# Tw6249/dgppo_fov

Hardware: AMD Instinct MI355X
Metric: env-steps/sec + PPO-updates/sec, LidarSpread n=8 ×4096 envs, 1/2/4/8 GPU (higher is better)
Workload: dtype f32; 1 GPU; LidarSpread n=8 obs=3 rays=32 top_k=8, 4096 envs/GPU, 1 step = reset + T=128 fused env steps into the (B,T+1) rollout buffer; env=LidarSpread, num_agents=8, n_obs=3, n_env_per_gpu=4096, T=128, hip_graph=True, stream_lanes=1, persistent_rollout=True, parallelism=dp1 (env-sharded, no collective)

## Files before the change

### dgppo_fov_amd/_lib.py

```python
from __future__ import annotations

import ctypes
import os
import pathlib

PKG_DIR = pathlib.Path(__file__).resolve().parent
LIB_PATH = pathlib.Path(os.environ.get("DGPPO_HIP_LIB", PKG_DIR / "lib" / "libdgppo_hip.so"))

DGPPO_EINVAL = -22
DGPPO_ENGINE_LIDAR, DGPPO_ENGINE_BICYCLE, DGPPO_ENGINE_MPE, DGPPO_ENGINE_OMNI = 0, 1, 2, 3
DGPPO_ENGINE_VMAS_WHEEL, DGPPO_ENGINE_VMAS_TRANSPORT = 4, 5
DGPPO_VMAS_FIELDS = 8
DGPPO_GOAL_SPREAD, DGPPO_GOAL_TARGET = 0, 1
(DGPPO_VARIANT_NONE, DGPPO_VARIANT_LINE, DGPPO_VARIANT_FORMATION, DGPPO_VARIANT_CORRIDOR,
 DGPPO_VARIANT_CONNECT) = 0, 1, 2, 3, 4
DGPPO_OBST_FIELDS = 16

c_f32p = ctypes.c_void_p


class NativeLibraryError(RuntimeError):
    pass


# ... 163 lines not shown

class GemmPlan(ctypes.Structure):
    _fields_ = [(n, ctypes.c_int32) for n in ("path", "form", "ntw", "ncg", "nch", "vec", "extra", "epi", "mt", "nt",
                                               "unroll", "flat", "pipe", "chunks", "split_k", "grid")] + \
               [("units", ctypes.c_int64), ("lds_bytes", ctypes.c_int64)]


class GruSeqArgs(ctypes.Structure):
    _fields_ = [
        ("Q", ctypes.c_int32), ("L", ctypes.c_int32), ("n_agents", ctypes.c_int32), ("H", ctypes.c_int32),
        ("gi", c_f32p), ("Wh", c_f32p), ("bhn", c_f32p), ("h0", c_f32p), ("hs", c_f32p), ("hT", c_f32p),
        ("dhs", c_f32p), ("dgi", c_f32p), ("dgh", c_f32p), ("dh0", c_f32p), ("dbhn_part", c_f32p),
    ]


class GtLayer(ctypes.Structure):
    _fields_ = [("Wq", c_f32p), ("bq", c_f32p), ("Wkt", c_f32p), ("bk", c_f32p), ("Wcat", c_f32p), ("Wu", c_f32p),
                ("bu", c_f32p), ("D", ctypes.c_int32), ("F", ctypes.c_int32), ("Wex", c_f32p)]


class PolicyStepArgs(ctypes.Structure):
    _fields_ = [
        ("G", ctypes.c_int32), ("N", ctypes.c_int32), ("E", ctypes.c_int32), ("n_agents", ctypes.c_int32),
        ("C", ctypes.c_int32), ("D0", ctypes.c_int32), ("A", ctypes.c_int32), ("n_layers", ctypes.c_int32),
        ("H", ctypes.c_int32), ("mode", ctypes.c_int32), ("ED", ctypes.c_int32), ("pad_", ctypes.c_int32),
        ("cand", c_f32p),
        ("nodes", c_f32p), ("nodes_gstride", ctypes.c_int64),
        ("edges", c_f32p), ("edges_gstride", ctypes.c_int64),
        ("receivers", c_f32p), ("senders", c_f32p), ("idx_gstride", ctypes.c_int64),
        ("layer", GtLayer * 2),
# ... 135 lines not shown
    "dgppo_policy_step_supported": (ctypes.c_int, [_V]),
    "dgppo_policy_work_floats": (ctypes.c_int64, []),
    "dgppo_policy_prepare": (ctypes.c_int, [_V, _V]),
    "dgppo_policy_step": (ctypes.c_int, [_V, _V]),
    "dgppo_gnn_sender_table": (ctypes.c_int, [_I32, _I32, _I32, _I32, _V, _V, _V, _V, _V]),
    "dgppo_cost_shaped_loss": (ctypes.c_int, [_V, _V, ctypes.c_float, _V, _I32, _I32, _I32, _I32, _V]),
    "dgppo_informarl_advantages": (ctypes.c_int, [_V, _V, _V, _I32, _I32, _I32, _V]),
    "dgppo_gnn_edge_wsum": (ctypes.c_int, [_I32, _I32, _I32, _I32, _I32, _I32, _V, _V, _V, _V, _V, _V]),
    "dgppo_gnn_edge_da": (ctypes.c_int, [_I32, _I32, _I32, _I32, _I32, _I32, _V, _V, _V, _V, _V, _V]),
    "dgppo_gru_seq_fwd": (ctypes.c_int, [_V, _V]),
    "dgppo_gru_seq_bwd": (ctypes.c_int, [_V, _V]),
    "dgppo_agent_mean_fwd": (ctypes.c_int, [_V, _V, _I64, _I32, _I32, _I64, _V]),
    "dgppo_agent_mean_bwd": (ctypes.c_int, [_V, _V, _I64, _I32, _I32, _I64, _V]),
    "dgppo_agent_mean_bwd_masked": (ctypes.c_int, [_V, _V, _V, _I64, _I32, _I32, _I64, _V]),
    "dgppo_gru_set_form": (ctypes.c_int, [_I32]),
    "dgppo_gnn_set_graph_otf": (ctypes.c_int, [_I32]),
    "dgppo_tanh_normal": (ctypes.c_int, [ctypes.POINTER(TanhNormalArgs), ctypes.c_void_p]),
    "dgppo_loss_workspace_floats": (ctypes.c_int64, []),
    "dgppo_ppo_loss": (ctypes.c_int, [_V, _V, _V, _V, _I64, _F32, _F32, _V, _V, _V, _V, _V]),
    "dgppo_l2_loss": (ctypes.c_int, [_V, _V, _I64, _V, _V, _V, _V]),
    "dgppo_gae": (ctypes.c_int, [ctypes.POINTER(GaeArgs), ctypes.c_void_p]),
    "dgppo_dgppo_advantages": (ctypes.c_int, [ctypes.POINTER(AdvArgs), ctypes.c_void_p]),
    "dgppo_grad_norm": (ctypes.c_int, [_V, _I64, _V, _V, _V]),
    "dgppo_adam": (ctypes.c_int, [_V, _V, _V, _V, _I64, _V, _F32, ctypes.c_double, ctypes.c_double, _F32, _F32, _V]),
    "dgppo_adam_multi_workspace_floats": (ctypes.c_int64, []),
    "dgppo_adam_multi": (ctypes.c_int, [_V, _V]),
    "dgppo_normal": (ctypes.c_int, [_V, _I64, _V, ctypes.c_uint64, ctypes.c_uint64, _V]),
    "dgppo_clip_min0": (ctypes.c_int, [_V, _V, _I64, _V]),
    "dgppo_lagr_advantages": (ctypes.c_int, [_V, _V, _V, _V, _V, _V, _V, _I32, _I32, _I32, _I32, _V]),
    "dgppo_lagr_update": (ctypes.c_int, [_V, _V, _V, _V, _V, _V, _I64, _I32, _I32, _F32, _F32, _V]),
# ... 62 lines not shown
```

### dgppo_fov_amd/algo/module/nets.py

```python
from __future__ import annotations

import ctypes
import math
import os

import numpy as np
import torch

from ... import _lib
from ...nn import kernels as K
from ...nn.layers import FUSE_LN, GNN, Dense, GraphBatch, MLPHead, ParamSpace, RNNStack

VH_TAIL = os.environ.get("DGPPO_VH_TAIL", "0") == "1"
STD_DEV_INIT_INV = math.log(math.exp(0.5) - 1.0)
STD_DEV_MIN = 1e-5


class _Net:
    modules: list

    def init_host(self, seed: int):
        rng = np.random.default_rng(seed)
        for m in self.modules:
            m.init_host(rng)

    @property
# ... 103 lines not shown
        feat, h2, _ = self.gru.fwd(y, h, h_out=h_out)
        _, mu, sr = self._outputs(feat)
        action = action_out if action_out is not None else torch.empty((rows, self.A), device=h.device)
        log_pi = log_pi_out if log_pi_out is not None else torch.empty(rows, device=h.device)
        a = _lib.TanhNormalArgs()
        a.rows, a.A, a.mode, a.n_agents = rows, self.A, mode, self.n
        a.mean, a.std_raw = K._p(mu), K._p(sr)
        a.std_shift, a.std_min = STD_DEV_INIT_INV, STD_DEV_MIN
        a.noise = K._p(noise)
        a.action_out, a.log_pi = K._p(action), K._p(log_pi)
        K.tanh_normal(a, h.device)
        return action, log_pi, h2

    def eval_seq_fwd(self, g: GraphBatch, S: int, L: int, actions: torch.Tensor, entropy_eps: torch.Tensor):
        n, dev = self.n, actions.device
        y, tc = self._trunk(g)
        H2, gcs = self.gru.seq_fwd(y, S * n, L, n)
        s, mu, sr = self._outputs(H2)
        rows = S * L * n
        log_pi = torch.empty(rows, device=dev)
        ent = torch.empty(rows, device=dev)
        a = _lib.TanhNormalArgs()
        a.rows, a.A, a.mode, a.n_agents = rows, self.A, 2, n
        a.mean, a.std_raw, a.action = K._p(mu), K._p(sr), K._p(actions)
        a.std_shift, a.std_min = STD_DEV_INIT_INV, STD_DEV_MIN
        a.log_pi, a.entropy, a.entropy_eps = K._p(log_pi), K._p(ent), K._p(entropy_eps)
        K.tanh_normal(a, dev)
        cache = (g, S, L, tc, gcs, H2, s, mu, sr, actions, entropy_eps)
        return log_pi, ent, cache

    def eval_seq_bwd(self, cache, dlog_pi, dentropy):
        g, S, L, tc, gcs, H2, s, mu, sr, actions, entropy_eps = cache
# ... 3 lines not shown
        dsr = torch.empty_like(sr)
        a = _lib.TanhNormalArgs()
        a.rows, a.A, a.mode, a.n_agents = rows, self.A, 2, n
        a.mean, a.std_raw, a.action = K._p(mu), K._p(sr), K._p(actions)
        a.std_shift, a.std_min = STD_DEV_INIT_INV, STD_DEV_MIN
        a.entropy_eps = K._p(entropy_eps)
        a.dlog_pi, a.dentropy, a.dmean, a.dstd_raw = K._p(dlog_pi), K._p(dentropy), K._p(dmu), K._p(dsr)
        K.tanh_normal(a, dev)
        ds = self.mean.bwd(s, dmu, rows)
        self.std.bwd(s, dsr, rows, dx_out=ds, accumulate=True)
        dH2 = self.scale_hid.bwd(H2, ds, rows)
        self._bptt(dH2.view(S, L, n, 64), gcs, S, L, tc, g)

    def _bptt(self, dHs, gcs, S, L, tc, g):
        gc, hc = tc
        ln = self.head.ln1_bwd_args(hc) if self.gru.simple else None
        dY, _ = self.gru.seq_bwd(gcs, dHs.reshape(S * L * self.n, 64), ln=ln)
        fused = ln is not None
        dz = self.head.bwd(hc, dY, dy_is_dh1=fused, mask_input=fused)
        self.gnn.bwd(gc, dz, g, top_masked=fused)


class VlNet(_Net):
    def __init__(self, node_dim: int, n_agents: int, device, seed: int = 1, gnn_layers: int = 2, edge_dim: int = 4,
                 rnn: str = "gru", rnn_layers: int = 1):
        self.n = n_agents
        ps = self.ps = ParamSpace()
        self.gnn = GNN(ps, "gnn", node_dim, gnn_layers, edge_dim=edge_dim)
        self.head = MLPHead(ps, "head")
        self.gru = RNNStack(ps, "gru", rnn, rnn_layers)
        self.out = Dense(ps, "out", 64, 1)
        self.modules = [self.gnn, self.head, self.gru, self.out]
        ps.build(device)
        self.init_host(seed)
# ... 13 lines not shown
        z, _ = self.gnn.fwd(g, keep=False)
        K.agent_mean_fwd(z, zm, g.G, self.n, 64, self.n * 64)
        return zm

    def seq_fwd(self, g: GraphBatch, S: int, L: int, h0=None, keep_cache=True, zm=None):
        dev = self.ps.flat.device
        G = S * L
        if zm is not None:
            assert not keep_cache, "seq_fwd from precomputed agent means is forward-only"
            z = gc = None
        else:
            n = self.n
            z, gc = self.gnn.fwd(g, keep=keep_cache)
            zm = torch.empty((G, 64), device=dev)
            K.agent_mean_fwd(z, zm, G, n, 64, n * 64)
        y, hc = self.head.fwd(zm)
        hT = torch.empty((S, self.gru.W), device=dev)
        Hs, gcs = self.gru.seq_fwd(y, S, L, 1, h0=h0, hT_out=hT)
        v = self.out.fwd(Hs, G)
        cache = (g, S, L, gc, z, hc, gcs, Hs) if keep_cache else None
        return v.view(S, L), hT, cache

    def seq_bwd(self, cache, dv):
        g, S, L, gc, z, hc, gcs, Hs = cache
        n, dev = self.n, dv.device
        G = S * L
        dH = self.out.bwd(Hs, dv.reshape(G, 1).contiguous(), G)
        ln = self.head.ln1_bwd_args(hc) if self.gru.simple else None
        dY, _ = self.gru.seq_bwd(gcs, dH, ln=ln)
        dzm = self.head.bwd(hc, dY, dy_is_dh1=ln is not None)
        dz = torch.empty_like(z)
        K.agent_mean_bwd(dzm, dz, G, n, 64, n * 64, mask=z if FUSE_LN else None)
        self.gnn.bwd(gc, dz, g, top_masked=FUSE_LN)


class VhNet(_Net):
    def __init__(self, node_dim: int, n_agents: int, n_cost: int, device, seed: int = 2, gnn_layers: int = 1,
                 edge_dim: int = 4, rnn: str = "gru", rnn_layers: int = 1):
        self.n, self.n_cost = n_agents, n_cost
        ps = self.ps = ParamSpace()
        self.gnn = GNN(ps, "gnn", node_dim, gnn_layers, edge_dim=edge_dim)
        self.head = MLPHead(ps, "head")
        self.gru = RNNStack(ps, "gru", rnn, rnn_layers)
        self.out = Dense(ps, "out", 64, n_cost)
        self.modules = [self.gnn, self.head, self.gru, self.out]
# ... 10 lines not shown

    def fwd(self, g: GraphBatch, h: torch.Tensor, keep_cache=True):
        rows = g.G * self.n
        self.last_tail = False
        if VH_TAIL and not keep_cache and self.gru.simple and len(self.gnn.layers) == 1 and h.shape[1] == 64:
            out = torch.empty((rows, self.n_cost), device=h.device)
            hd, cell = self.head, self.gru.cells[0]
            v = self.ps.view
            tail_w = [hd.d0.W(), hd.d0.b(), v(hd.ln0.name + ".scale"), v(hd.ln0.name + ".bias"), hd.d1.W(), hd.d1.b(),
                      v(hd.ln1.name + ".scale"), v(hd.ln1.name + ".bias"), cell.v("Wi"), cell.v("bi"), cell.v("Wh"),
                      cell.v("bhn"), self.out.W(), self.out.b()]
            if self.gnn.fwd_epilogue(g, tail=(tail_w, h if h.is_contiguous() else h.contiguous(), out)) is not None:
                self.last_tail = True
                return out, None
        z, gc = self.gnn.fwd(g, keep=keep_cache)
        y, hc = self.head.fwd(z)
        h2, _, rc = self.gru.fwd(y, h)
        out = self.out.fwd(h2, rows)
        return out, ((g, gc, hc, rc, h2) if keep_cache else None)

    def bwd(self, cache, dout):
        g, gc, hc, rc, h2 = cache
        rows = g.G * self.n
        dh2 = self.out.bwd(h2, dout, rows)
        ln = self.head.ln1_bwd_args(hc) if self.gru.simple else None
        dy, _ = self.gru.seq_bwd(rc, dh2, ln=ln)
        fused = ln is not None
        dz = self.head.bwd(hc, dy, dy_is_dh1=fused, mask_input=fused)
        self.gnn.bwd(gc, dz, g, top_masked=fused)


class VhGlobalNet(_Net):

    def __init__(self, node_dim: int, n_agents: int, n_cost: int, device, seed: int = 2, gnn_layers: int = 1,
                 edge_dim: int = 4, rnn: str = "gru", rnn_layers: int = 1):
        self.n, self.n_cost = n_agents, n_cost
        ps = self.ps = ParamSpace()
        self.gnn = GNN(ps, "gnn", node_dim, gnn_layers, edge_dim=edge_dim)
        self.head = MLPHead(ps, "head", d_in=128)
        self.gru = RNNStack(ps, "gru", rnn, rnn_layers)
        self.out = Dense(ps, "out", 64, n_cost)
        self.modules = [self.gnn, self.head, self.gru, self.out]
        ps.build(device)
# ... 54 lines not shown
```

### dgppo_fov_amd/csrc/gemm.hip

```cpp
#include <hip/hip_runtime.h>
#include <stdint.h>
#include <stdlib.h>

#include "../../include/dgppo_hip.h"
#include "lanes.h"
#include "lds_attr.h"

namespace dgppo {

typedef float f32x16 __attribute__((ext_vector_type(16)));

constexpr int kBM = 64, kBN = 64, kBK = 32, kPitch = kBM + 1;

__device__ float4 g_zero_row[4];
__device__ float g_sink[64];

struct GemmTileArgs {
  int M, N, K, k_begin, k_end;
  bool ta, tb;
  const float* A;
  int64_t lda;
  const float* B;
  int64_t ldb;
  int a_grp, b_grp;
// ... 148 lines not shown
struct EpiAcc {
  float ds[NTW], db[NTW];
};

__device__ __forceinline__ float swz16(float v) {
  return __builtin_bit_cast(float, __builtin_amdgcn_ds_swizzle(__builtin_bit_cast(int, v), 0x401F));
}
__device__ __forceinline__ float red32(float v) {
  v = lanes::sum16(v);
  return v + swz16(v);
}
__device__ __forceinline__ void ln_stats(float v0, float v1, float& mean, float& rstd) {
#pragma clang fp contract(off)
  const float s1 = red32(v0 + v1);
  const float s2 = red32(v0 * v0 + v1 * v1);
  mean = s1 / 64.0f;
  float var = s2 / 64.0f - mean * mean;
  var = var > 0.0f ? var : 0.0f;
  rstd = 1.0f / sqrtf(var + 1e-6f);
}
__device__ __forceinline__ float ln_pre(float v, float mean, float rstd, float sc, float bi) {
#pragma clang fp contract(off)
  return ((v - mean) * rstd) * sc + bi;
}

template <int NTW, int EXTRA, int EPI>
__device__ __forceinline__ void epi_load(const dgppo_gemm_args& p, const float* C, const float* Dd, int m0, int col0,
                                         int i, int h, float (&bv)[NTW], float (&xv)[NTW][16], EpiX<NTW, EPI>& ex) {
#pragma clang fp contract(off)
  if (EPI == dgppo::kEpiLnBwd) {
    const int row = m0 + (i & 3) + 8 * ((i & 15) >> 2) + 4 * h;
    const bool ok = row < p.M;
    ex.mo = *(ok ? p.ln_mean + row : (const float*)g_zero_row);
    ex.ro = *(ok ? p.ln_rstd + row : (const float*)g_zero_row);
  }
#pragma unroll
  for (int t = 0; t < NTW; ++t) {
    const int col = col0 + 32 * t + i;
// ... 1179 lines not shown
```

### dgppo_fov_amd/nn/kernels.py

```python
from __future__ import annotations

import ctypes
import math
import weakref

import torch

from .. import _lib, ops

_WS = {}
_GRAPHS = weakref.WeakSet()
_WS_KEPT = []


def hold_for_graph(g):
    _GRAPHS.add(g)
    return g


def workspace(nfloats: int, device, slot: str = "default") -> torch.Tensor:
    key = (str(device), slot, _lib.stream_handle(device))
    t = _WS.get(key)
    if t is None or t.numel() < nfloats:
        old = t.numel() if t is not None else 0
# ... 212 lines not shown
    a = _lib.GruSeqArgs()
    a.Q, a.L, a.n_agents, a.H = int(Q), int(L), int(n), 64
    a.gi, a.Wh, a.bhn, a.h0, a.hs, a.hT = _p(gi), _p(Wh), _p(bhn), _p(h0), _p(hs), _p(hT)
    a.dhs, a.dgi, a.dgh, a.dh0, a.dbhn_part = _p(dhs), _p(dgi), _p(dgh), _p(dh0), _p(dbhn_part)
    lib = _lib.load()
    if fwd:
        _chk(lib.dgppo_gru_seq_fwd(ctypes.byref(a), _stream(hs)), "dgppo_gru_seq_fwd")
    else:
        _chk(lib.dgppo_gru_seq_bwd(ctypes.byref(a), _stream(hs)), "dgppo_gru_seq_bwd")


def gru_seq_blocks(Q):
    return int(_lib.load().dgppo_gru_seq_blocks(int(Q)))


def agent_mean_fwd(x, y, G, n, F, x_gstride):
    _chk(_lib.load().dgppo_agent_mean_fwd(_p(x), _p(y), int(G), int(n), int(F), int(x_gstride), _stream(y)),
         "dgppo_agent_mean_fwd")


def agent_mean_bwd(dy, dx, G, n, F, dx_gstride, mask=None):
    _chk(_lib.load().dgppo_agent_mean_bwd_masked(_p(dy), _p(mask), _p(dx), int(G), int(n), int(F), int(dx_gstride),
                                                 _stream(dx)), "dgppo_agent_mean_bwd_masked")


def sender_table(G, n, C, E, cand, receivers, senders, out):
    _chk(_lib.load().dgppo_gnn_sender_table(int(G), int(n), int(C), int(E), _p(cand), _p(receivers), _p(senders),
                                            _p(out), _stream(out)), "dgppo_gnn_sender_table")


# ... 99 lines not shown
```

### dgppo_fov_amd/nn/layers.py

```python
from __future__ import annotations

import math
import os
from typing import Dict, List, Optional, Tuple

import numpy as np
import torch

from .. import ops
from . import kernels as K

FUSE_LN = os.environ.get("DGPPO_FUSE_LN", "1") == "1"
FUSED_LAYER = os.environ.get("DGPPO_FUSED_LAYER", "1") == "1"


class ParamSpace:

    def __init__(self):
        self.entries: List[Tuple[str, Tuple[int, ...], str]] = []
        self.offsets: Dict[str, int] = {}
        self.size = 0
        self.flat = None
        self.grad = None

    def add(self, name: str, shape, init: str) -> str:
        shape = tuple(int(s) for s in shape)
        assert name not in self.offsets, name
        self.offsets[name] = self.size
# ... 222 lines not shown
        H = self.H
        wi, bi, wh, bhn = (self.v(k).cpu().numpy() for k in ("Wi", "bi", "Wh", "bhn"))
        return {"ir": {"kernel": wi[:, :H], "bias": bi[:H]}, "iz": {"kernel": wi[:, H:2 * H], "bias": bi[H:2 * H]},
                "in": {"kernel": wi[:, 2 * H:], "bias": bi[2 * H:]}, "hr": {"kernel": wh[:, :H]},
                "hz": {"kernel": wh[:, H:2 * H]}, "hn": {"kernel": wh[:, 2 * H:], "bias": bhn}}

    def load_flax(self, d):
        wi = np.concatenate([d["ir"]["kernel"], d["iz"]["kernel"], d["in"]["kernel"]], 1).astype(np.float32)
        bi = np.concatenate([d["ir"]["bias"], d["iz"]["bias"], d["in"]["bias"]]).astype(np.float32)
        wh = np.concatenate([d["hr"]["kernel"], d["hz"]["kernel"], d["hn"]["kernel"]], 1).astype(np.float32)
        self.v("Wi").copy_(torch.from_numpy(wi))
        self.v("bi").copy_(torch.from_numpy(bi))
        self.v("Wh").copy_(torch.from_numpy(wh))
        self.v("bhn").copy_(torch.as_tensor(np.asarray(d["hn"]["bias"], np.float32)))

    def seq_fwd(self, x, Q, L, n, h0=None, hs_out=None, hT_out=None):
        rows, H = Q * L, self.H
        gi = torch.empty((rows, 3 * H), device=x.device)
        K.gemm(x, self.v("Wi"), gi, rows, 3 * H, self.d_in, bias=self.v("bi"))
        hs = hs_out if hs_out is not None else torch.empty((rows, H), device=x.device)
        K.gru_seq(True, Q, L, n, gi, self.v("Wh"), self.v("bhn"), h0, hs, hT=hT_out)
        return hs, (x, gi, hs, h0, Q, L, n)

    def seq_bwd(self, cache, dhs, need_dx=True, need_dh0=False, ln=None):
        x, gi, hs, h0, Q, L, n = cache
        rows, H, dev = Q * L, self.H, dhs.device
        dgi = torch.empty((rows, 3 * H), device=dev)
        dgh = torch.empty((rows, 3 * H), device=dev)
        dh0 = torch.empty((Q, H), device=dev) if need_dh0 else None
        nb = K.gru_seq_blocks(Q)
        part = K.workspace(nb * H, dev, "gru_bhn")
        K.gru_seq(False, Q, L, n, gi, self.v("Wh"), self.v("bhn"), h0, hs, dhs=dhs, dgi=dgi, dgh=dgh, dh0=dh0,
                  dbhn_part=part)
        K.gemm(x, dgi, self.v("Wi", True), self.d_in, 3 * H, rows, ta=True, beta=1.0, bias_grad=self.v("bi", True))
        S = Q // n
        if L > 1:
            K.gemm(hs, dgh, self.v("Wh", True), H, 3 * H, S * (L - 1) * n, ta=True, lda=H, a_grp=(L - 1) * n,
                   a_gs=L * n * H, ldb=3 * H, b_off=n * 3 * H, b_grp=(L - 1) * n, b_gs=L * n * 3 * H, beta=1.0)
        if h0 is not None:
            K.gemm(h0, dgh, self.v("Wh", True), H, 3 * H, Q, ta=True, lda=H, ldb=3 * H, b_grp=n,
                   b_gs=L * n * 3 * H, beta=1.0)
        K.colsum(part, nb, H, self.v("bhn", True), beta=1.0)
        dx = None
        if need_dx:
            dx = torch.empty_like(x)
            K.gemm(dgi, self.v("Wi"), dx, rows, self.d_in, 3 * H, tb=True, ldb=3 * H, ln=ln)
        return dx, dh0

    def fwd(self, x, h, h_out=None):
        rows = h.shape[0]
        return self.seq_fwd(x, rows, 1, 1, h0=h, hs_out=h_out)

    def bwd(self, cache, dhn, need_dx=True):
        return self.seq_bwd(cache, dhn, need_dx=need_dx, need_dh0=True)


class LSTMCell:
# ... 162 lines not shown
            dh0s.append(dh0k)
        dh0 = torch.cat(dh0s[::-1], 1) if need_dh0 else None
        return d, dh0

    def fwd(self, x, h, h_out=None):
        rows = h.shape[0]
        if self.simple:
            h2, c = self.cells[0].fwd(x, h, h_out=h_out)
            return h2, h2, c
        h2 = h_out if h_out is not None else torch.empty((rows, self.W), device=h.device)
        y, c = self.seq_fwd(x, rows, 1, 1, h0=h, hT_out=h2)
        return y, h2, c

    def bwd(self, cache, dy, need_dx=True, ln=None):
        return self.seq_bwd(cache, dy, need_dx=need_dx, need_dh0=True, ln=ln)


class GraphTransformer:

    def __init__(self, ps, name, D, F, H=3, ED=4):
        self.ps, self.name, self.D, self.F, self.H = ps, name, D, F, H
        self.ED, self.EX = ED, ED - 4
        if ED < 4:
            raise ValueError(f"edge_dim {ED} < 4")
        ps.add(name + ".Wq", (D, H * F), "orthogonal")
        ps.add(name + ".bq", (H * F,), "zeros")
        ps.add(name + ".Wkt", (H, F, D), "orthogonal")
        ps.add(name + ".bk", (H * F,), "zeros")
        ps.add(name + ".Wcat", (H * (D + 5), F), "orthogonal")
        ps.add(name + ".Wu", (D, F), "orthogonal")
# ... 413 lines not shown
```

### include/dgppo_hip.h

```cpp
#ifndef DGPPO_HIP_H
#define DGPPO_HIP_H

#include <stdint.h>

#ifdef __cplusplus
extern "C" {
#endif

#define DGPPO_ABI_VERSION 14
#define DGPPO_EINVAL (-22)

#define DGPPO_ENGINE_LIDAR 0
#define DGPPO_ENGINE_BICYCLE 1
#define DGPPO_ENGINE_MPE 2
#define DGPPO_ENGINE_OMNI 3
#define DGPPO_ENGINE_VMAS_WHEEL 4
#define DGPPO_ENGINE_VMAS_TRANSPORT 5
#define DGPPO_GOAL_SPREAD 0
#define DGPPO_GOAL_TARGET 1
#define DGPPO_VARIANT_NONE 0
#define DGPPO_VARIANT_LINE 1
#define DGPPO_VARIANT_FORMATION 2
#define DGPPO_VARIANT_CORRIDOR 3
#define DGPPO_VARIANT_CONNECT 4
// ... 287 lines not shown
  const float* h0;
  float* hs;
  float* hT;
  const float* dhs;
  float* dgi;
  float* dgh;
  float* dh0;
  float* dbhn_part;
} dgppo_gru_seq_args;

int64_t dgppo_gru_seq_blocks(int32_t Q);
int dgppo_gru_seq_fwd(const dgppo_gru_seq_args* args, void* stream);
int dgppo_gru_seq_bwd(const dgppo_gru_seq_args* args, void* stream);
int dgppo_gru_set_form(int32_t regb);

typedef struct dgppo_gt_layer {
  const float *Wq, *bq, *Wkt, *bk, *Wcat, *Wu, *bu;
  int32_t D, F;
  const float* Wex;
} dgppo_gt_layer;

typedef struct dgppo_policy_step_args {
  int32_t G, N, E, n_agents, C, D0, A, n_layers, H, mode;
  int32_t ED, pad_;
  const int32_t* cand;
  const float* nodes; int64_t nodes_gstride;
  const float* edges; int64_t edges_gstride;
  const int32_t* receivers;
  const int32_t* senders; int64_t idx_gstride;
  dgppo_gt_layer layer[2];
// ... 132 lines not shown
```

Measured before the change: 446.8 million env-steps/s.

## Fuse MLP head (two dense+LN+ReLU) and GRU input GEMM into one MFMA kernel

Adds a persistent HIP kernel that runs both 64x64 dense layers with LayerNorm+ReLU and the GRU input projection for a row tile in registers, with the weights staged in LDS, writing only gi and optional training caches. A matching backward kernel chains the dgi->dy1->dh1->dy0->dh0->dz transposed GEMMs and the LN backward passes, with per-block partials for the LN parameter gradients. This removes several kernel launches and global round trips of intermediate activations in the actor/critic forward and backward paths. The new path is gated by shape checks and an env flag, and the rollout policy step may already use its own fused path, so env-step throughput may not change.

```diff
diff --git a/dgppo_fov_amd/_lib.py b/dgppo_fov_amd/_lib.py
--- a/dgppo_fov_amd/_lib.py
+++ b/dgppo_fov_amd/_lib.py
@@ -201,6 +201,19 @@
     ]
 
 
+class HeadChainArgs(ctypes.Structure):
+    _fields_ = [("rows", ctypes.c_int64)] + \
+               [(n, c_f32p) for n in ("x", "W0", "b0", "ln0_s", "ln0_b", "W1", "b1", "ln1_s", "ln1_b", "Wi", "bi", "gi",
+                                      "h0", "h1", "mean0", "rstd0", "mean1", "rstd1", "y0", "y1")]
+
+
+class HeadChainBwdArgs(ctypes.Structure):
+    _fields_ = [("rows", ctypes.c_int64)] + \
+               [(n, c_f32p) for n in ("dgi", "x", "h0", "h1", "mean0", "rstd0", "mean1", "rstd1", "W0", "ln0_s", "ln0_b",
+                                      "W1", "ln1_s", "ln1_b", "Wi", "dz", "dh0", "dh1", "ln_part")] + \
+               [("mask_input", ctypes.c_int32)]
+
+
 class GtLayer(ctypes.Structure):
     _fields_ = [("Wq", c_f32p), ("bq", c_f32p), ("Wkt", c_f32p), ("bk", c_f32p), ("Wcat", c_f32p), ("Wu", c_f32p),
                 ("bu", c_f32p), ("D", ctypes.c_int32), ("F", ctypes.c_int32), ("Wex", c_f32p)]
@@ -366,6 +379,11 @@
     "dgppo_agent_mean_bwd": (ctypes.c_int, [_V, _V, _I64, _I32, _I32, _I64, _V]),
     "dgppo_agent_mean_bwd_masked": (ctypes.c_int, [_V, _V, _V, _I64, _I32, _I32, _I64, _V]),
     "dgppo_gru_set_form": (ctypes.c_int, [_I32]),
+    "dgppo_head_chain_supported": (ctypes.c_int, [ctypes.POINTER(HeadChainArgs)]),
+    "dgppo_head_chain_blocks": (ctypes.c_int64, [_I64]),
+    "dgppo_head_chain_fwd": (ctypes.c_int, [ctypes.POINTER(HeadChainArgs), ctypes.c_void_p]),
+    "dgppo_head_chain_bwd_supported": (ctypes.c_int, [ctypes.POINTER(HeadChainBwdArgs)]),
+    "dgppo_head_chain_bwd": (ctypes.c_int, [ctypes.POINTER(HeadChainBwdArgs), ctypes.c_void_p]),
     "dgppo_gnn_set_graph_otf": (ctypes.c_int, [_I32]),
     "dgppo_tanh_normal": (ctypes.c_int, [ctypes.POINTER(TanhNormalArgs), ctypes.c_void_p]),
     "dgppo_loss_workspace_floats": (ctypes.c_int64, []),
diff --git a/dgppo_fov_amd/algo/module/nets.py b/dgppo_fov_amd/algo/module/nets.py
--- a/dgppo_fov_amd/algo/module/nets.py
+++ b/dgppo_fov_amd/algo/module/nets.py
@@ -9,7 +9,7 @@
 
 from ... import _lib
 from ...nn import kernels as K
-from ...nn.layers import FUSE_LN, GNN, Dense, GraphBatch, MLPHead, ParamSpace, RNNStack
+from ...nn.layers import FUSE_LN, GNN, Dense, GraphBatch, MLPHead, ParamSpace, RNNStack, head_rnn_bwd, head_rnn_fwd
 
 VH_TAIL = os.environ.get("DGPPO_VH_TAIL", "0") == "1"
 STD_DEV_INIT_INV = math.log(math.exp(0.5) - 1.0)
@@ -143,8 +143,9 @@
 
     def eval_seq_fwd(self, g: GraphBatch, S: int, L: int, actions: torch.Tensor, entropy_eps: torch.Tensor):
         n, dev = self.n, actions.device
-        y, tc = self._trunk(g)
-        H2, gcs = self.gru.seq_fwd(y, S * n, L, n)
+        z, gc = self.gnn.fwd(g)
+        H2, hc, gcs = head_rnn_fwd(self.head, self.gru, z, S * n, L, n)
+        tc = (gc, hc)
         s, mu, sr = self._outputs(H2)
         rows = S * L * n
         log_pi = torch.empty(rows, device=dev)
@@ -178,10 +179,7 @@
 
     def _bptt(self, dHs, gcs, S, L, tc, g):
         gc, hc = tc
-        ln = self.head.ln1_bwd_args(hc) if self.gru.simple else None
-        dY, _ = self.gru.seq_bwd(gcs, dHs.reshape(S * L * self.n, 64), ln=ln)
-        fused = ln is not None
-        dz = self.head.bwd(hc, dY, dy_is_dh1=fused, mask_input=fused)
+        dz, fused = head_rnn_bwd(self.head, self.gru, hc, gcs, dHs.reshape(S * L * self.n, 64), mask_input=True)
         self.gnn.bwd(gc, dz, g, top_masked=fused)
 
 
@@ -225,9 +223,8 @@
             z, gc = self.gnn.fwd(g, keep=keep_cache)
             zm = torch.empty((G, 64), device=dev)
             K.agent_mean_fwd(z, zm, G, n, 64, n * 64)
-        y, hc = self.head.fwd(zm)
         hT = torch.empty((S, self.gru.W), device=dev)
-        Hs, gcs = self.gru.seq_fwd(y, S, L, 1, h0=h0, hT_out=hT)
+        Hs, hc, gcs = head_rnn_fwd(self.head, self.gru, zm, S, L, 1, h0=h0, hT_out=hT, keep=keep_cache)
         v = self.out.fwd(Hs, G)
         cache = (g, S, L, gc, z, hc, gcs, Hs) if keep_cache else None
         return v.view(S, L), hT, cache
@@ -237,9 +234,7 @@
         n, dev = self.n, dv.device
         G = S * L
         dH = self.out.bwd(Hs, dv.reshape(G, 1).contiguous(), G)
-        ln = self.head.ln1_bwd_args(hc) if self.gru.simple else None
-        dY, _ = self.gru.seq_bwd(gcs, dH, ln=ln)
-        dzm = self.head.bwd(hc, dY, dy_is_dh1=ln is not None)
+        dzm, _ = head_rnn_bwd(self.head, self.gru, hc, gcs, dH)
         dz = torch.empty_like(z)
         K.agent_mean_bwd(dzm, dz, G, n, 64, n * 64, mask=z if FUSE_LN else None)
         self.gnn.bwd(gc, dz, g, top_masked=FUSE_LN)
@@ -280,8 +275,11 @@
                 self.last_tail = True
                 return out, None
         z, gc = self.gnn.fwd(g, keep=keep_cache)
-        y, hc = self.head.fwd(z)
-        h2, _, rc = self.gru.fwd(y, h)
+        if self.gru.simple:
+            h2, hc, rc = head_rnn_fwd(self.head, self.gru, z, rows, 1, 1, h0=h, keep=keep_cache)
+        else:
+            y, hc = self.head.fwd(z)
+            h2, _, rc = self.gru.fwd(y, h)
         out = self.out.fwd(h2, rows)
         return out, ((g, gc, hc, rc, h2) if keep_cache else None)
 
@@ -289,10 +287,7 @@
         g, gc, hc, rc, h2 = cache
         rows = g.G * self.n
         dh2 = self.out.bwd(h2, dout, rows)
-        ln = self.head.ln1_bwd_args(hc) if self.gru.simple else None
-        dy, _ = self.gru.seq_bwd(rc, dh2, ln=ln)
-        fused = ln is not None
-        dz = self.head.bwd(hc, dy, dy_is_dh1=fused, mask_input=fused)
+        dz, fused = head_rnn_bwd(self.head, self.gru, hc, rc, dh2, mask_input=True)
         self.gnn.bwd(gc, dz, g, top_masked=fused)
 
 
diff --git a/dgppo_fov_amd/csrc/gemm.hip b/dgppo_fov_amd/csrc/gemm.hip
--- a/dgppo_fov_amd/csrc/gemm.hip
+++ b/dgppo_fov_amd/csrc/gemm.hip
@@ -5,6 +5,7 @@
 #include "../../include/dgppo_hip.h"
 #include "lanes.h"
 #include "lds_attr.h"
+#include "ln_row.h"
 
 namespace dgppo {
 
@@ -186,14 +187,7 @@
 #pragma clang fp contract(off)
   const float s1 = red32(v0 + v1);
   const float s2 = red32(v0 * v0 + v1 * v1);
-  mean = s1 / 64.0f;
-  float var = s2 / 64.0f - mean * mean;
-  var = var > 0.0f ? var : 0.0f;
-  rstd = 1.0f / sqrtf(var + 1e-6f);
-}
-__device__ __forceinline__ float ln_pre(float v, float mean, float rstd, float sc, float bi) {
-#pragma clang fp contract(off)
-  return ((v - mean) * rstd) * sc + bi;
+  ln_finish(s1, s2, mean, rstd);
 }
 
 template <int NTW, int EXTRA, int EPI>
diff --git a/dgppo_fov_amd/csrc/head_chain.hip b/dgppo_fov_amd/csrc/head_chain.hip
--- /dev/null
+++ b/dgppo_fov_amd/csrc/head_chain.hip
@@ -0,0 +1,394 @@
+#include <hip/hip_runtime.h>
+#include <stdint.h>
+
+#include "../../include/dgppo_hip.h"
+#include "lanes.h"
+#include "lds_attr.h"
+#include "ln_row.h"
+
+namespace dgppo {
+
+typedef float hc_f32x16 __attribute__((ext_vector_type(16)));
+
+constexpr int kHcThreads = 512, kHcWaves = kHcThreads / 64;
+constexpr int kHcCUs = 256;
+constexpr int kHcW0 = 0, kHcW1 = 4096, kHcWi = 8192, kHcVec = 20480, kHcLds = kHcVec + 6 * 64 + 192;
+
+__device__ __forceinline__ int hc_feat(int t, int r, int h) { return 32 * t + 8 * (r >> 2) + 4 * h + (r & 3); }
+
+__device__ __forceinline__ void hc_load_row(const float* src, int h, float (&v)[4][8]) {
+#pragma unroll
+  for (int c = 0; c < 4; ++c) {
+    const float4 a = *(const float4*)(src + 16 * c + 8 * h), b = *(const float4*)(src + 16 * c + 8 * h + 4);
+    v[c][0] = a.x, v[c][1] = a.y, v[c][2] = a.z, v[c][3] = a.w;
+    v[c][4] = b.x, v[c][5] = b.y, v[c][6] = b.z, v[c][7] = b.w;
+  }
+}
+
+__device__ __forceinline__ void hc_store_row(float* dst, int h, const float (&v)[2][16]) {
+#pragma unroll
+  for (int t = 0; t < 2; ++t)
+#pragma unroll
+    for (int j = 0; j < 4; ++j)
+      *(float4*)(dst + 32 * t + 8 * j + 4 * h) = make_float4(v[t][4 * j], v[t][4 * j + 1], v[t][4 * j + 2], v[t][4 * j + 3]);
+}
+
+__device__ __forceinline__ void hc_ln_relu(const hc_f32x16 (&acc)[2], const float* vec, int h, float (&hv)[2][16],
+                                           float (&y)[2][16], float& mean, float& rstd) {
+#pragma clang fp contract(off)
+  float s1 = 0.0f, s2 = 0.0f;
+#pragma unroll
+  for (int t = 0; t < 2; ++t)
+#pragma unroll
+    for (int r = 0; r < 16; ++r) {
+      const float v = acc[t][r] + vec[hc_feat(t, r, h)];
+      hv[t][r] = v;
+      s1 += v;
+      s2 += v * v;
+    }
+  s1 += __shfl_xor(s1, 32, 64);
+  s2 += __shfl_xor(s2, 32, 64);
+  ln_finish(s1, s2, mean, rstd);
+#pragma unroll
+  for (int t = 0; t < 2; ++t)
+#pragma unroll
+    for (int r = 0; r < 16; ++r) {
+      const int f = hc_feat(t, r, h);
+      const float p = ln_pre(hv[t][r], mean, rstd, vec[64 + f], vec[128 + f]);
+      y[t][r] = p > 0.0f ? p : 0.0f;
+    }
+}
+
+template <int NT, int LD>
+__device__ __forceinline__ void hc_gemm_acc(const float* W, int i, int h, const float (&y)[2][16],
+                                            hc_f32x16 (&acc)[NT]) {
+#pragma unroll
+  for (int t = 0; t < 2; ++t)
+#pragma unroll
+    for (int r = 0; r < 16; ++r) {
+      const float* wr = W + hc_feat(t, r, h) * LD + i;
+#pragma unroll
+      for (int mo = 0; mo < NT; ++mo) acc[mo] = __builtin_amdgcn_mfma_f32_32x32x2f32(wr[32 * mo], y[t][r], acc[mo], 0, 0, 0);
+    }
+}
+
+template <int NT>
+__device__ __forceinline__ void hc_zero(hc_f32x16 (&acc)[NT]) {
+#pragma unroll
+  for (int t = 0; t < NT; ++t)
+#pragma unroll
+    for (int r = 0; r < 16; ++r) acc[t][r] = 0.0f;
+}
+
+__global__ __launch_bounds__(kHcThreads) void head_chain_fwd_kernel(dgppo_head_chain_args p) {
+  extern __shared__ __attribute__((aligned(16))) float lds[];
+  const int lane = threadIdx.x & 63, wave = threadIdx.x >> 6;
+  const int i = lane & 31, h = lane >> 5;
+  const int64_t units = (p.rows + 31) / 32;
+  const int64_t ustep = (int64_t)gridDim.x * kHcWaves;
+  int64_t u = blockIdx.x + (int64_t)gridDim.x * wave;
+  auto row_of = [&](int64_t uu, bool& ok) -> int64_t {
+    const int64_t row = uu * 32 + i;
+    ok = row < p.rows;
+    return ok ? row : 0;
+  };
+  bool rok;
+  int64_t row = row_of(u, rok);
+  float xv[4][8];
+  hc_load_row(p.x + row * 64, h, xv);
+  {
+    auto stage = [&](const float* src, int dst, int n4) {
+      for (int e = threadIdx.x; e < n4; e += kHcThreads) *(float4*)(lds + dst + 4 * e) = *(const float4*)(src + 4 * e);
+    };
+    stage(p.W0, kHcW0, 1024);
+    stage(p.W1, kHcW1, 1024);
+    stage(p.Wi, kHcWi, 3072);
+    stage(p.b0, kHcVec, 16);
+    stage(p.ln0_s, kHcVec + 64, 16);
+    stage(p.ln0_b, kHcVec + 128, 16);
+    stage(p.b1, kHcVec + 192, 16);
+    stage(p.ln1_s, kHcVec + 256, 16);
+    stage(p.ln1_b, kHcVec + 320, 16);
+    stage(p.bi, kHcVec + 384, 48);
+  }
+  __syncthreads();
+  for (; u < units; u += ustep) {
+    hc_f32x16 acc[2];
+    hc_zero<2>(acc);
+#pragma unroll
+    for (int c = 0; c < 4; ++c)
+#pragma unroll
+      for (int q = 0; q < 8; ++q) {
+        const float* wr = lds + kHcW0 + (16 * c + 8 * h + q) * 64 + i;
+#pragma unroll
+        for (int mo = 0; mo < 2; ++mo) acc[mo] = __builtin_amdgcn_mfma_f32_32x32x2f32(wr[32 * mo], xv[c][q], acc[mo], 0, 0, 0);
+      }
+    const int64_t orow = row;
+    const bool ook = rok;
+    row = row_of(u + ustep, rok);
+    hc_load_row(p.x + row * 64, h, xv);
+    float hv[2][16], y[2][16], mean, rstd;
+    hc_ln_relu(acc, lds + kHcVec, h, hv, y, mean, rstd);
+    if (ook) {
+      if (p.h0) {
+        hc_store_row(p.h0 + orow * 64, h, hv);
+        if (h == 0) p.mean0[orow] = mean, p.rstd0[orow] = rstd;
+      }
+      if (p.y0) hc_store_row(p.y0 + orow * 64, h, y);
+    }
+    hc_zero<2>(acc);
+    hc_gemm_acc<2, 64>(lds + kHcW1, i, h, y, acc);
+    hc_ln_relu(acc, lds + kHcVec + 192, h, hv, y, mean, rstd);
+    if (ook) {
+      if (p.h1) {
+        hc_store_row(p.h1 + orow * 64, h, hv);
+        if (h == 0) p.mean1[orow] = mean, p.rstd1[orow] = rstd;
+      }
+      if (p.y1) hc_store_row(p.y1 + orow * 64, h, y);
+    }
+    hc_f32x16 g[6];
+    hc_zero<6>(g);
+    hc_gemm_acc<6, 192>(lds + kHcWi, i, h, y, g);
+    if (ook) {
+      const float* bi = lds + kHcVec + 384;
+      float* dst = p.gi + orow * 192;
+#pragma unroll
+      for (int t = 0; t < 6; ++t)
+#pragma unroll
+        for (int j = 0; j < 4; ++j) {
+          const int f = 32 * t + 8 * j + 4 * h;
+          *(float4*)(dst + f) = make_float4(g[t][4 * j] + bi[f], g[t][4 * j + 1] + bi[f + 1], g[t][4 * j + 2] + bi[f + 2],
+                                            g[t][4 * j + 3] + bi[f + 3]);
+        }
+    }
+  }
+}
+
+constexpr int kHbW0 = 0, kHbW1 = 64 * 65, kHbWi = 2 * 64 * 65, kHbVec = kHbWi + 64 * 193, kHbLds = kHbVec + 256;
+
+__device__ __forceinline__ void hc_load_acc_row(const float* src, int h, float (&v)[2][16]) {
+#pragma unroll
+  for (int t = 0; t < 2; ++t)
+#pragma unroll
+    for (int j = 0; j < 4; ++j) {
+      const float4 a = *(const float4*)(src + 32 * t + 8 * j + 4 * h);
+      v[t][4 * j] = a.x, v[t][4 * j + 1] = a.y, v[t][4 * j + 2] = a.z, v[t][4 * j + 3] = a.w;
+    }
+}
+
+template <int LD>
+__device__ __forceinline__ void hc_gemm_t_acc(const float* W, int i, int h, const float (&d)[2][16], hc_f32x16 (&acc)[2]) {
+#pragma unroll
+  for (int t = 0; t < 2; ++t)
+#pragma unroll
+    for (int r = 0; r < 16; ++r) {
+      const float* wr = W + i * LD + hc_feat(t, r, h);
+#pragma unroll
+      for (int mo = 0; mo < 2; ++mo) acc[mo] = __builtin_amdgcn_mfma_f32_32x32x2f32(wr[32 * mo * LD], d[t][r], acc[mo], 0, 0, 0);
+    }
+}
+
+__device__ __forceinline__ void hc_ln_bwd(const hc_f32x16 (&dy)[2], const float* hrow, float mean, float rstd,
+                                          const float* vec, int h, bool ok, float (&dh)[2][16], float& pds,
+                                          float& pdb) {
+#pragma clang fp contract(off)
+  float xh[2][16], g[2][16];
+  hc_load_acc_row(hrow, h, xh);
+  float s1 = 0.0f, s2 = 0.0f;
+#pragma unroll
+  for (int t = 0; t < 2; ++t)
+#pragma unroll
+    for (int r = 0; r < 16; ++r) {
+      const int f = hc_feat(t, r, h);
+      const float hv = xh[t][r], d = ok ? dy[t][r] : 0.0f;
+      g[t][r] = ln_pre(hv, mean, rstd, vec[f], vec[64 + f]) > 0.0f ? d : 0.0f;
+      xh[t][r] = (hv - mean) * rstd;
+      const float gx = g[t][r] * vec[f];
+      s1 += gx;
+      s2 += gx * xh[t][r];
+    }
+  s1 += __shfl_xor(s1, 32, 64);
+  s2 += __shfl_xor(s2, 32, 64);
+  s1 = s1 / 64.0f;
+  s2 = s2 / 64.0f;
+  float red[32];
+  int cnt;
+#pragma unroll
+  for (int t = 0; t < 2; ++t)
+#pragma unroll
+    for (int r = 0; r < 16; ++r) red[16 * t + r] = g[t][r];
+  lanes::treduce32<32>(red, cnt);
+  pdb += red[0];
+#pragma unroll
+  for (int t = 0; t < 2; ++t)
+#pragma unroll
+    for (int r = 0; r < 16; ++r) red[16 * t + r] = g[t][r] * xh[t][r];
+  lanes::treduce32<32>(red, cnt);
+  pds += red[0];
+#pragma unroll
+  for (int t = 0; t < 2; ++t)
+#pragma unroll
+    for (int r = 0; r < 16; ++r) {
+      const float gx = g[t][r] * vec[hc_feat(t, r, h)];
+      dh[t][r] = rstd * ((gx - s1) - xh[t][r] * s2);
+    }
+}
+
+__global__ __launch_bounds__(kHcThreads) void head_chain_bwd_kernel(dgppo_head_chain_bwd_args p) {
+  extern __shared__ __attribute__((aligned(16))) float lds[];
+  const int lane = threadIdx.x & 63, wave = threadIdx.x >> 6;
+  const int i = lane & 31, h = lane >> 5;
+  const int64_t units = (p.rows + 31) / 32;
+  const int64_t ustep = (int64_t)gridDim.x * kHcWaves;
+  int64_t u = blockIdx.x + (int64_t)gridDim.x * wave;
+  auto row_of = [&](int64_t uu, bool& ok) -> int64_t {
+    const int64_t row = uu * 32 + i;
+    ok = row < p.rows;
+    return ok ? row : 0;
+  };
+  bool rok;
+  int64_t row = row_of(u, rok);
+  float dv[4][8];
+  hc_load_row(p.dgi + row * 192, h, dv);
+  {
+    auto stage = [&](const float* src, int dst, int ncol, int pitch) {
+      const int n4 = ncol / 4;
+      for (int e = threadIdx.x; e < 64 * n4; e += kHcThreads) {
+        const int k = e / n4, n = 4 * (e - k * n4);
+        const float4 a = *(const float4*)(src + k * ncol + n);
+        float* d = lds + dst + k * pitch + n;
+        d[0] = a.x, d[1] = a.y, d[2] = a.z, d[3] = a.w;
+      }
+    };
+    stage(p.W0, kHbW0, 64, 65);
+    stage(p.W1, kHbW1, 64, 65);
+    stage(p.Wi, kHbWi, 192, 193);
+    if (threadIdx.x < 64) {
+      lds[kHbVec + threadIdx.x] = p.ln1_s[threadIdx.x];
+      lds[kHbVec + 64 + threadIdx.x] = p.ln1_b[threadIdx.x];
+      lds[kHbVec + 128 + threadIdx.x] = p.ln0_s[threadIdx.x];
+      lds[kHbVec + 192 + threadIdx.x] = p.ln0_b[threadIdx.x];
+    }
+  }
+  __syncthreads();
+  float part[4] = {0.0f, 0.0f, 0.0f, 0.0f};
+  for (; u < units; u += ustep) {
+    hc_f32x16 acc[2];
+    hc_zero<2>(acc);
+    const float* drow = p.dgi + row * 192;
+#pragma unroll
+    for (int gq = 0; gq < 3; ++gq) {
+      float dn[4][8];
+      if (gq < 2) hc_load_row(drow + 64 * (gq + 1), h, dn);
+#pragma unroll
+      for (int c = 0; c < 4; ++c)
+#pragma unroll
+        for (int q = 0; q < 8; ++q) {
+          const float* wr = lds + kHbWi + i * 193 + 64 * gq + 16 * c + 8 * h + q;
+#pragma unroll
+          for (int mo = 0; mo < 2; ++mo)
+            acc[mo] = __builtin_amdgcn_mfma_f32_32x32x2f32(wr[32 * mo * 193], dv[c][q], acc[mo], 0, 0, 0);
+        }
+      if (gq < 2) {
+#pragma unroll
+        for (int c = 0; c < 4; ++c)
+#pragma unroll
+          for (int q = 0; q < 8; ++q) dv[c][q] = dn[c][q];
+      }
+    }
+    const int64_t orow = row;
+    const bool ook = rok;
+    __builtin_amdgcn_sched_barrier(0);
+    float dh[2][16];
+    hc_ln_bwd(acc, p.h1 + orow * 64, p.mean1[orow], p.rstd1[orow], lds + kHbVec, h, ook, dh, part[0], part[1]);
+    __builtin_amdgcn_sched_barrier(0);
+    if (ook && p.dh1) hc_store_row(p.dh1 + orow * 64, h, dh);
+    hc_zero<2>(acc);
+    hc_gemm_t_acc<65>(lds + kHbW1, i, h, dh, acc);
+    __builtin_amdgcn_sched_barrier(0);
+    hc_ln_bwd(acc, p.h0 + orow * 64, p.mean0[orow], p.rstd0[orow], lds + kHbVec + 128, h, ook, dh, part[2], part[3]);
+    __builtin_amdgcn_sched_barrier(0);
+    if (ook && p.dh0) hc_store_row(p.dh0 + orow * 64, h, dh);
+    hc_zero<2>(acc);
+    hc_gemm_t_acc<65>(lds + kHbW0, i, h, dh, acc);
+    __builtin_amdgcn_sched_barrier(0);
+    if (p.mask_input) {
+      float xm[2][16];
+      hc_load_acc_row(p.x + orow * 64, h, xm);
+#pragma unroll
+      for (int t = 0; t < 2; ++t)
+#pragma unroll
+        for (int r = 0; r < 16; ++r) dh[t][r] = xm[t][r] > 0.0f ? acc[t][r] : 0.0f;
+    } else {
+#pragma unroll
+      for (int t = 0; t < 2; ++t)
+#pragma unroll
+        for (int r = 0; r < 16; ++r) dh[t][r] = acc[t][r];
+    }
+    if (ook) hc_store_row(p.dz + orow * 64, h, dh);
+    __builtin_amdgcn_sched_barrier(0);
+    row = row_of(u + ustep, rok);
+    hc_load_row(p.dgi + row * 192, h, dv);
+  }
+  const int base = ((i & 8) ? 16 : 0) + ((i & 4) ? 8 : 0) + ((i & 2) ? 4 : 0) + ((i & 1) ? 2 : 0) + ((i & 16) ? 1 : 0);
+  const int f = hc_feat(base >> 4, base & 15, h);
+  __syncthreads();
+#pragma unroll
+  for (int q = 0; q < 4; ++q) lds[wave * 256 + 64 * q + f] = part[q];
+  __syncthreads();
+  if (threadIdx.x < 256) {
+    float v = lds[threadIdx.x];
+#pragma unroll
+    for (int w = 1; w < kHcWaves; ++w) v += lds[w * 256 + threadIdx.x];
+    p.ln_part[(int64_t)blockIdx.x * 256 + threadIdx.x] = v;
+  }
+}
+
+inline bool hc_aligned(const void* q) { return ((uintptr_t)q & 15) == 0; }
+
+}
+
+extern "C" int dgppo_head_chain_supported(const dgppo_head_chain_args* p) {
+  if (!p || p->rows < 1 || p->rows > (int64_t)1 << 40) return 0;
+  const void* need[] = {p->x, p->W0, p->b0, p->ln0_s, p->ln0_b, p->W1, p->b1, p->ln1_s, p->ln1_b, p->Wi, p->bi, p->gi};
+  for (const void* q : need)
+    if (!q || !dgppo::hc_aligned(q)) return 0;
+  const void* opt[] = {p->h0, p->h1, p->y0, p->y1};
+  for (const void* q : opt)
+    if (!dgppo::hc_aligned(q)) return 0;
+  const int n = !!p->h0 + !!p->h1 + !!p->mean0 + !!p->rstd0 + !!p->mean1 + !!p->rstd1;
+  return n == 0 || n == 6;
+}
+
+extern "C" int64_t dgppo_head_chain_blocks(int64_t rows) {
+  const int64_t units = (rows + 31) / 32;
+  return units < 1 ? 1 : (units < dgppo::kHcCUs ? units : dgppo::kHcCUs);
+}
+
+extern "C" int dgppo_head_chain_fwd(const dgppo_head_chain_args* p, void* stream) {
+  if (!dgppo_head_chain_supported(p)) return DGPPO_EINVAL;
+  dgppo::allow_lds((const void*)dgppo::head_chain_fwd_kernel);
+  hipLaunchKernelGGL(dgppo::head_chain_fwd_kernel, dim3((unsigned)dgppo_head_chain_blocks(p->rows)),
+                     dim3(dgppo::kHcThreads), dgppo::kHcLds * sizeof(float), (hipStream_t)stream, *p);
+  return (int)hipGetLastError();
+}
+
+extern "C" int dgppo_head_chain_bwd_supported(const dgppo_head_chain_bwd_args* p) {
+  if (!p || p->rows < 1 || p->rows > (int64_t)1 << 40) return 0;
+  const void* need[] = {p->dgi, p->h0, p->h1, p->W0, p->W1, p->Wi, p->dz, p->mean0, p->rstd0, p->mean1, p->rstd1,
+                        p->ln0_s, p->ln0_b, p->ln1_s, p->ln1_b, p->ln_part};
+  for (const void* q : need)
+    if (!q) return 0;
+  const void* al[] = {p->dgi, p->h0, p->h1, p->W0, p->W1, p->Wi, p->dz, p->x, p->dh0, p->dh1};
+  for (const void* q : al)
+    if (!dgppo::hc_aligned(q)) return 0;
+  return p->mask_input ? p->x != nullptr : 1;
+}
+
+extern "C" int dgppo_head_chain_bwd(const dgppo_head_chain_bwd_args* p, void* stream) {
+  if (!dgppo_head_chain_bwd_supported(p)) return DGPPO_EINVAL;
+  dgppo::allow_lds((const void*)dgppo::head_chain_bwd_kernel);
+  hipLaunchKernelGGL(dgppo::head_chain_bwd_kernel, dim3((unsigned)dgppo_head_chain_blocks(p->rows)),
+                     dim3(dgppo::kHcThreads), dgppo::kHbLds * sizeof(float), (hipStream_t)stream, *p);
+  return (int)hipGetLastError();
+}
diff --git a/dgppo_fov_amd/csrc/ln_row.h b/dgppo_fov_amd/csrc/ln_row.h
--- /dev/null
+++ b/dgppo_fov_amd/csrc/ln_row.h
@@ -0,0 +1,18 @@
+#pragma once
+#include <hip/hip_runtime.h>
+
+namespace dgppo {
+
+__device__ __forceinline__ void ln_finish(float s1, float s2, float& mean, float& rstd) {
+#pragma clang fp contract(off)
+  mean = s1 / 64.0f;
+  float var = s2 / 64.0f - mean * mean;
+  var = var > 0.0f ? var : 0.0f;
+  rstd = 1.0f / sqrtf(var + 1e-6f);
+}
+__device__ __forceinline__ float ln_pre(float v, float mean, float rstd, float sc, float bi) {
+#pragma clang fp contract(off)
+  return ((v - mean) * rstd) * sc + bi;
+}
+
+}
diff --git a/dgppo_fov_amd/nn/kernels.py b/dgppo_fov_amd/nn/kernels.py
--- a/dgppo_fov_amd/nn/kernels.py
+++ b/dgppo_fov_amd/nn/kernels.py
@@ -250,6 +250,57 @@
     return int(_lib.load().dgppo_gru_seq_blocks(int(Q)))
 
 
+CHAIN_LOG = None
+
+HEAD_CHAIN_TILE = 32
+
+
+def head_chain_blocks(rows) -> int:
+    return int(_lib.load().dgppo_head_chain_blocks(int(rows)))
+
+
+def head_chain_fwd(x, W0, b0, ln0_s, ln0_b, W1, b1, ln1_s, ln1_b, Wi, bi, gi, train=None, y0=None, y1=None) -> bool:
+    lib = _lib.load()
+    _lib.require_gpu(gi.device, "head_chain_fwd")
+    a = _lib.HeadChainArgs()
+    a.rows = int(x.shape[0])
+    a.x, a.W0, a.b0, a.ln0_s, a.ln0_b = _p(x), _p(W0), _p(b0), _p(ln0_s), _p(ln0_b)
+    a.W1, a.b1, a.ln1_s, a.ln1_b, a.Wi, a.bi, a.gi = _p(W1), _p(b1), _p(ln1_s), _p(ln1_b), _p(Wi), _p(bi), _p(gi)
+    if train is not None:
+        a.h0, a.h1, a.mean0, a.rstd0, a.mean1, a.rstd1 = (_p(t) for t in train)
+    a.y0, a.y1 = _p(y0), _p(y1)
+    if not lib.dgppo_head_chain_supported(ctypes.byref(a)):
+        return False
+    if CHAIN_LOG is not None:
+        CHAIN_LOG.append((a.rows, train is not None))
+    _chk(lib.dgppo_head_chain_fwd(ctypes.byref(a), _stream(gi)), "dgppo_head_chain_fwd")
+    return True
+
+
+def head_chain_bwd(dgi, x, h0, h1, stats, W0, ln0_s, ln0_b, W1, ln1_s, ln1_b, Wi, dz, dh0, dh1, dln0, dln1,
+                   mask_input=False):
+    lib = _lib.load()
+    _lib.require_gpu(dz.device, "head_chain_bwd")
+    a = _lib.HeadChainBwdArgs()
+    a.rows = int(dgi.shape[0])
+    a.dgi, a.x, a.h0, a.h1 = _p(dgi), _p(x), _p(h0), _p(h1)
+    a.mean0, a.rstd0, a.mean1, a.rstd1 = (_p(t) for t in stats)
+    a.W0, a.ln0_s, a.ln0_b, a.W1, a.ln1_s, a.ln1_b, a.Wi = (_p(t) for t in (W0, ln0_s, ln0_b, W1, ln1_s, ln1_b, Wi))
+    a.dz, a.dh0, a.dh1, a.mask_input = _p(dz), _p(dh0), _p(dh1), int(mask_input)
+    nb = head_chain_blocks(a.rows)
+    part = workspace(nb * 256, dz.device, "head_chain_ln")
+    a.ln_part = _p(part)
+    if CHAIN_LOG is not None:
+        CHAIN_LOG.append((a.rows, "bwd"))
+    _chk(lib.dgppo_head_chain_bwd(ctypes.byref(a), _stream(dz)), "dgppo_head_chain_bwd")
+    for off, (ds, db) in ((0, dln1), (128, dln0)):
+        if db.data_ptr() == ds.data_ptr() + 4 * 64:
+            colsum(part, nb, 128, ds, ld=256, x_off=off, beta=1.0)
+        else:
+            colsum(part, nb, 64, ds, ld=256, x_off=off, beta=1.0)
+            colsum(part, nb, 64, db, ld=256, x_off=off + 64, beta=1.0)
+
+
 def agent_mean_fwd(x, y, G, n, F, x_gstride):
     _chk(_lib.load().dgppo_agent_mean_fwd(_p(x), _p(y), int(G), int(n), int(F), int(x_gstride), _stream(y)),
          "dgppo_agent_mean_fwd")
diff --git a/dgppo_fov_amd/nn/layers.py b/dgppo_fov_amd/nn/layers.py
--- a/dgppo_fov_amd/nn/layers.py
+++ b/dgppo_fov_amd/nn/layers.py
@@ -12,6 +12,7 @@
 
 FUSE_LN = os.environ.get("DGPPO_FUSE_LN", "1") == "1"
 FUSED_LAYER = os.environ.get("DGPPO_FUSED_LAYER", "1") == "1"
+HEAD_CHAIN = os.environ.get("DGPPO_HEAD_CHAIN", "1") == "1"
 
 
 class ParamSpace:
@@ -264,15 +265,16 @@
         self.v("Wh").copy_(torch.from_numpy(wh))
         self.v("bhn").copy_(torch.as_tensor(np.asarray(d["hn"]["bias"], np.float32)))
 
-    def seq_fwd(self, x, Q, L, n, h0=None, hs_out=None, hT_out=None):
+    def seq_fwd(self, x, Q, L, n, h0=None, hs_out=None, hT_out=None, gi=None):
         rows, H = Q * L, self.H
-        gi = torch.empty((rows, 3 * H), device=x.device)
-        K.gemm(x, self.v("Wi"), gi, rows, 3 * H, self.d_in, bias=self.v("bi"))
-        hs = hs_out if hs_out is not None else torch.empty((rows, H), device=x.device)
+        if gi is None:
+            gi = torch.empty((rows, 3 * H), device=x.device)
+            K.gemm(x, self.v("Wi"), gi, rows, 3 * H, self.d_in, bias=self.v("bi"))
+        hs = hs_out if hs_out is not None else torch.empty((rows, H), device=gi.device)
         K.gru_seq(True, Q, L, n, gi, self.v("Wh"), self.v("bhn"), h0, hs, hT=hT_out)
         return hs, (x, gi, hs, h0, Q, L, n)
 
-    def seq_bwd(self, cache, dhs, need_dx=True, need_dh0=False, ln=None):
+    def seq_bwd(self, cache, dhs, need_dx=True, need_dh0=False, ln=None, ret_dgi=False):
         x, gi, hs, h0, Q, L, n = cache
         rows, H, dev = Q * L, self.H, dhs.device
         dgi = torch.empty((rows, 3 * H), device=dev)
@@ -291,6 +293,8 @@
             K.gemm(h0, dgh, self.v("Wh", True), H, 3 * H, Q, ta=True, lda=H, ldb=3 * H, b_grp=n,
                    b_gs=L * n * 3 * H, beta=1.0)
         K.colsum(part, nb, H, self.v("bhn", True), beta=1.0)
+        if ret_dgi:
+            return dgi, dh0
         dx = None
         if need_dx:
             dx = torch.empty_like(x)
@@ -483,6 +487,53 @@
 
     def bwd(self, cache, dy, need_dx=True, ln=None):
         return self.seq_bwd(cache, dy, need_dx=need_dx, need_dh0=True, ln=ln)
+
+
+def head_rnn_fwd(head: MLPHead, rnn: RNNStack, x, Q, L, n, h0=None, hs_out=None, hT_out=None, keep=True):
+    cell = rnn.cells[0] if rnn.simple else None
+    if HEAD_CHAIN and FUSE_LN and cell is not None and cell.d_in == 64 and cell.H == 64 and x.is_contiguous() and \
+            (head.d0.d_in, head.d0.d_out, head.d1.d_in, head.d1.d_out) == (64, 64, 64, 64):
+        rows, dev = x.shape[0], x.device
+        v = head.d0.ps.view
+        gi = torch.empty((rows, 192), device=dev)
+        train = y0 = y1 = None
+        if keep:
+            h0r, h1r, y0, y1 = (torch.empty((rows, 64), device=dev) for _ in range(4))
+            m0, r0, m1, r1 = (torch.empty(rows, device=dev) for _ in range(4))
+            train = (h0r, h1r, m0, r0, m1, r1)
+        if K.head_chain_fwd(x, head.d0.W(), head.d0.b(), v(head.ln0.name + ".scale"), v(head.ln0.name + ".bias"),
+                            head.d1.W(), head.d1.b(), v(head.ln1.name + ".scale"), v(head.ln1.name + ".bias"),
+                            cell.v("Wi"), cell.v("bi"), gi, train=train, y0=y0, y1=y1):
+            hc = (x, y0, (h0r, y0, m0, r0, "fused"), (h1r, y1, m1, r1, "chain")) if keep else None
+            hs, rc = cell.seq_fwd(y1, Q, L, n, h0=h0, hs_out=hs_out, hT_out=hT_out, gi=gi)
+            return hs, hc, (rc if keep else None)
+    y, hc = head.fwd(x)
+    hs, rc = rnn.seq_fwd(y, Q, L, n, h0=h0, hs_out=hs_out, hT_out=hT_out)
+    return hs, hc, rc
+
+
+def head_rnn_bwd(head: MLPHead, rnn: RNNStack, hc, rc, dhs, mask_input=False):
+    cell = rnn.cells[0] if rnn.simple else None
+    x, y0, c0, c1 = hc
+    if HEAD_CHAIN and FUSE_LN and cell is not None and cell.d_in == 64 and cell.H == 64 and len(c0) == 5 and \
+            len(c1) == 5 and c1[4] == "chain" and x.is_contiguous() and \
+            (head.d0.d_in, head.d0.d_out, head.d1.d_in, head.d1.d_out) == (64, 64, 64, 64):
+        rows, dev = x.shape[0], x.device
+        dgi, _ = cell.seq_bwd(rc, dhs, ret_dgi=True)
+        dz, dh0, dh1 = (torch.empty((rows, 64), device=dev) for _ in range(3))
+        v = head.d0.ps.view
+        n0, n1 = head.ln0.name, head.ln1.name
+        K.head_chain_bwd(dgi, x, c0[0], c1[0], (c0[2], c0[3], c1[2], c1[3]), head.d0.W(), v(n0 + ".scale"),
+                         v(n0 + ".bias"), head.d1.W(), v(n1 + ".scale"), v(n1 + ".bias"), cell.v("Wi"), dz, dh0, dh1,
+                         (v(n0 + ".scale", True), v(n0 + ".bias", True)), (v(n1 + ".scale", True), v(n1 + ".bias", True)),
+                         mask_input=mask_input)
+        head.d1.bwd(y0, dh1, rows, need_dx=False)
+        head.d0.bwd(x, dh0, rows, need_dx=False)
+        return dz, True
+    ln = head.ln1_bwd_args(hc) if rnn.simple else None
+    dY, _ = rnn.seq_bwd(rc, dhs, ln=ln)
+    fused = ln is not None
+    return head.bwd(hc, dY, dy_is_dh1=fused, mask_input=fused and mask_input), fused
 
 
 class GraphTransformer:
diff --git a/include/dgppo_hip.h b/include/dgppo_hip.h
--- a/include/dgppo_hip.h
+++ b/include/dgppo_hip.h
@@ -325,6 +325,39 @@
 int dgppo_gru_seq_bwd(const dgppo_gru_seq_args* args, void* stream);
 int dgppo_gru_set_form(int32_t regb);
 
+typedef struct dgppo_head_chain_args {
+  int64_t rows;
+  const float* x;
+  const float *W0, *b0;
+  const float *ln0_s, *ln0_b;
+  const float *W1, *b1;
+  const float *ln1_s, *ln1_b;
+  const float *Wi, *bi;
+  float* gi;
+  float *h0, *h1;
+  float *mean0, *rstd0, *mean1, *rstd1;
+  float *y0, *y1;
+} dgppo_head_chain_args;
+
+int dgppo_head_chain_supported(const dgppo_head_chain_args* args);
+int64_t dgppo_head_chain_blocks(int64_t rows);
+int dgppo_head_chain_fwd(const dgppo_head_chain_args* args, void* stream);
+
+typedef struct dgppo_head_chain_bwd_args {
+  int64_t rows;
+  const float* dgi;
+  const float *x, *h0, *h1;
+  const float *mean0, *rstd0, *mean1, *rstd1;
+  const float *W0, *ln0_s, *ln0_b, *W1, *ln1_s, *ln1_b, *Wi;
+  float* dz;
+  float *dh0, *dh1;
+  float* ln_part;
+  int32_t mask_input;
+} dgppo_head_chain_bwd_args;
+
+int dgppo_head_chain_bwd_supported(const dgppo_head_chain_bwd_args* args);
+int dgppo_head_chain_bwd(const dgppo_head_chain_bwd_args* args, void* stream);
+
 typedef struct dgppo_gt_layer {
   const float *Wq, *bq, *Wkt, *bk, *Wcat, *Wu, *bu;
   int32_t D, F;
```

Result: no change. 445.1 million env-steps/s (-0.4%).
